# Ascend-Research/HeadPoseEstimation-WHENet

Measured on AMD Instinct MI355X. Metric: head crops/sec (224x224), higher is better.
Workload: dtype f16

## Files before the change

headposeestimation-whenet_amd/csrc/engine.cpp:

```cpp
#include "engine_internal.h"

#include <mutex>

#include <algorithm>
#include <cstdlib>
#include <cmath>
#include <cstring>

namespace whenet {

using namespace detail;

void* Engine::upload_bytes(const void* p, size_t nbytes) {
    weight_allocs_.emplace_back();
    weight_allocs_.back().reset(nbytes);
    void* d = weight_allocs_.back().as<void>();
    if (nbytes) WHENET_HIP_CHECK(hipMemcpy(d, p, nbytes, hipMemcpyHostToDevice));
    return d;
}

template <typename T> T* Engine::upload(const std::vector<T>& v) {
    return static_cast<T*>(upload_bytes(v.data(), v.size() * sizeof(T)));
}

// ... 170 lines not shown
        head_fuse_ = value != 0;
    } else if (key == "concurrent") {
        xcd_always_ = value != 0;
    } else if (key == "xcd_map") {
        WHENET_REQUIRE(value >= 0 && value <= 7, WHENET_EINVAL, "xcd_map must be a bit mask 0..7 (1 = front / front2, 2 = front7, 4 = head7)");
        xcd_map_ = int(value);
    } else if (key == "mb7") {
        mb7_ = value != 0;
    } else if (key == "front7") {
        front7_ = value != 0;
    } else if (key == "fold12") {
        fold12_ = value != 0;
    } else if (key == "front2_static") {
        WHENET_REQUIRE(value == 0 || value == 1, WHENET_EINVAL, "front2_static must be 0 (runtime tile geometry everywhere) or 1 (per layer, default)");
        front2_static_ = value != 0;
    } else if (key == "front_static") {
        WHENET_REQUIRE(value == 0 || value == 1, WHENET_EINVAL, "front_static must be 0 (runtime tile geometry everywhere) or 1 (per layer, default)");
        front_static_ = value != 0;
    } else if (key == "pw_static") {
        WHENET_REQUIRE(value == 0 || value == 1, WHENET_EINVAL, "pw_static must be 0 (runtime layer shapes everywhere) or 1 (per layer, default)");
        pw_static_ = value != 0;
    } else if (key == "stem_fuse") {
        stem_fuse_ = value != 0;
    } else if (key == "act_layout") {
        WHENET_REQUIRE(value >= 0 && value <= 2, WHENET_EINVAL,
                       "act_layout must be 0 (NHWC everywhere), 1 (16-channel blocks per layer, default) or 2 (16-channel blocks wherever supported)");
        act_layout_ = int(value);
    } else if (key == "poison") {
        poison_ = value != 0;
        return;
// ... 231 lines not shown
    } else {
        const DevBlock& c = blocks_[size_t(index)];
        const BlockSchedule cs = block_schedule(c);
        if (cs.use_mb7 || !cs.use_f7) return false;
        if (c.spec.has_skip() && c.project.K < 320) return false;
    }
    static constexpr bool WINS[17] = {false, false, false, false, false, false, false, false, false, false, false, false,
                                      true, true, true, true, true};
    return act_layout_ == 2 || (index <= 16 && WINS[index]);
}

bool Engine::front2_static(int index) const {
    static constexpr bool WINS[17] = {false, false, true, true, true, true, false, true, true, true, true, true, true,
                                      false, false, false, false};
    return front2_static_ && index >= 0 && index <= 16 && WINS[index];
}

bool Engine::pw_static(int index) const {
    static constexpr bool WINS[17] = {false, false, true, true, true, false, false, true, false, true, false, false, false,
                                      true, true, true, true};
    return pw_static_ && se_fuse_ == 1 && index >= 0 && index <= 16 && WINS[index];
}

bool Engine::front_static(int index) const {
    static constexpr bool WINS[17] = {false, false, false, false, false, false, true, false, false, false, false, false, false,
                                      false, false, false, false};
    return front_static_ && index >= 0 && index <= 16 && WINS[index];
}

void* Engine::enqueue_blocks(int first, int last, const View& v, void* cur, int n, hipStream_t s, LaunchRecorder* rec,
// ... 109 lines not shown
        fill_front_tiled(a, b);
        a.wep = b.expand.wp;
        a.wdt = b.dw.wt;
        if (fold == 2) {
            a.wep = d_fold12_w32_;
            a.be = fold12_pw_.bias;
            a.Cin = fold12_pw_.K;
            a.KSe = fold12_pw_.KS;
            a.NTe = fold12_pw_.NTILES;
            a.in_gate = static_cast<const float*>(v.gate);
        }
        a.xcd_grouped = xcd_grouped(1, n);
        a.plan = b.f2plan;
        a.plan.threads = front2_threads(b.f2plan, n);
        a.static_form = front2_static(sp.index);
        R(p + "/front", "front",
          kernel_name_front2(sp.k, sp.s, a.KSe, a.plan.threads, a.plan.xs, a.in_gate != nullptr, front2_static_row(a)).c_str(),
          bytes(a.Cin), flops(a.Cin), [&] { launch_front2(a, s); });
    } else if (bs.use_f2s) {
        Front2sArgs a{};
        fill_front_common(a, b, v, in, n);
        fill_front_tiled(a, b);
        a.weps = b.expand.wps;
        a.wdt = b.dw.wts;
        a.KSe = b.expand.KSs;
        a.wsi = b.expand.wsi;
        a.wsi_d = b.dw.wts_wsi;
        a.tm = b.f2s_tm;
        a.plan = b.f2splan;
        R(p + "/front", "front", kernel_name_front2s(sp.k, sp.s, a.KSe, a.plan.threads, a.tm, false).c_str(), bytes(a.Cin),
          flops(a.Cin), [&] { launch_front2s(a, s); });
    } else {
// ... 594 lines not shown
```

headposeestimation-whenet_amd/csrc/engine.h:

```cpp
#pragma once

#include <deque>
#include <map>
#include <memory>
#include <string>
#include <tuple>
#include <utility>
#include <vector>

#include "common.h"
#include "kernels.h"
#include "snapshot.h"

namespace whenet {

template <typename H, hipError_t (*Destroy)(H)>
class Owned {
  public:
    Owned() = default;
    Owned(Owned&& o) noexcept : h_(o.h_) { o.h_ = nullptr; }
    ~Owned() { reset(); }
    void reset() {
        if (h_) (void)Destroy(h_);
        h_ = nullptr;
// ... 357 lines not shown
    void enqueue_project(const DevBlock& b, const SeFuse& sef, bool se_fused, const View& v, const void* in, void* out, int n,
                         hipStream_t s, LaunchRecorder* rec, bool in_blocked, bool out_blocked);
    template <typename A> void fill_front_common(A& a, const DevBlock& b, const View& v, const void* in, int n) const;
    Head7Args head7_args(const void* x, float* feat, int n) const;
    PwArgs head_pw_args(const void* x, void* out, int n) const { return pw_args(head_, x, out, n * 49, 49, ACT_SWISH); }
    void* enqueue_blocks(int first, int last, const View& v, void* cur, int n, hipStream_t s, LaunchRecorder* rec,
                         bool b1_dw_done = false);
    bool stem_fuse_active() const;
    bool fold12_active() const;
    bool head_fused() const;
    bool heads_split_active() const;
    void launch_heads_stage(const HeadsArgs& h, const View& v, hipStream_t s);
    bool act_blocked(int index) const;
    bool front_static(int index) const;
    bool pw_static(int index) const;
    bool front2_static(int index) const;
    int act_layout_ = 1;
    struct BlockSchedule {
        bool fused = false, use_f2 = false, use_f2s = false, use_f7 = false, se_in_front = false, se_fused = false, se_mfma = false;
        bool use_mb7 = false;
        int se_ntiles = 1, se_chunks = 1;
    };
    BlockSchedule block_schedule(const DevBlock& b, int n = 0) const;
    int se_fuse_tiny_ = 0;
    int f2s_mask_ = -1;
    bool single_stage_call_ = false;
    bool range_call_ = false;
    int lanes_for(int n, int want) const;
    template <typename F> void for_each_lane(int n, int lanes, hipStream_t s, F&& body);
    void enqueue_lanes(const uint8_t* d_in, int n, Results out, hipStream_t s, int want = 0);
// ... 96 lines not shown
    bool fuse_front_ = true;
    int se_fuse_ = 1;
    int front_impl_ = 1;
    bool poison_ = false;
    bool head_fuse_ = true;
    bool front7_ = true;
    bool mb7_ = false;
    int xcd_map_ = 7;
    bool xcd_always_ = false;
    bool xcd_grouped(int bit, int n) const {
        return (xcd_map_ & bit) != 0 && (xcd_always_ || n >= 128);
    }
    bool stem_fuse_ = true;
    bool front_static_ = true;
    bool pw_static_ = true;
    bool front2_static_ = true;
    bool fold12_ = true;
    int lanes_ = 2;
    bool lane_graphs_ = false;
    int min_lane_crops_ = 16;
    int host_lanes_ = 2;
    Stream stream_, copy_stream_;
    std::vector<Stream> lane_streams_;
    std::vector<Event> join_ev_;
    Event fork_ev_;
    hipDeviceProp_t prop_{};
    int64_t params_backbone_ = 0, params_heads_ = 0;
    int n_tensors_ = 0;

    std::vector<DeviceBuffer> weight_allocs_;
// ... 60 lines not shown
```

headposeestimation-whenet_amd/csrc/front2.hip:

```cpp
#include "device_math.h"
#include "kernels.h"
#include "stamps.h"

#include <atomic>
#include <cstdlib>
#include <string>
#include <vector>

namespace whenet {

namespace {

constexpr int RL = 7;

__device__ __forceinline__ int fdiv2(int q, float rinv) { return int((float(q) + 0.5f) * rinv); }

struct F2Params {
    const half_t* x;
    const half_t* wep;
    const float* be;
    const half_t* wdt;
    const float* bd;
    half_t* out;
    float* rpart;
// ... 48 lines not shown
    g.chunks = cdiv(t.Cexp, g.CC);
    g.EH = (t.TH - 1) * t.s + t.k;
    g.EWp = 4 * (t.s * (t.TXG - 1) + nch);
    g.RP = g.EWp * 2;
    int cp = g.EH * g.RP + 8;
    cp = (cp + 63) / 64 * 64;
    g.CP = (cp - 32 >= g.EH * g.RP + 8) ? cp - 32 : cp + 32;
    const int ncq = cdiv((t.TH / RL) * t.TXG, 4);
    g.off_stage = (g.CC * g.CP + 15) & ~15;
    g.off_red = g.off_stage + (t.threads / 64) * 2048;
    g.off_sum = g.off_red + ncq * g.CC * 4;
    g.lds_bytes = g.off_sum + g.CC * 4;
    return g;
}

template <bool EDGE>
__device__ __forceinline__ void expand_store(const float16v& acc, float bias, unsigned char* ep, const int (&eoff)[4],
                                             const int (&drd)[4], const int (&dcd)[4], int nr_left, int ng_left) {
    (void)bias;
#pragma unroll
    for (int qq = 0; qq < 4; ++qq) {
        if (!EDGE || (drd[qq] < nr_left && dcd[qq] < ng_left)) {
            const float2v y0 = swish2(float2v{acc[4 * qq], acc[4 * qq + 1]});
            const float2v y1 = swish2(float2v{acc[4 * qq + 2], acc[4 * qq + 3]});
            half4 o;
            o[0] = half_t(y0[0]);
            o[1] = half_t(y0[1]);
            o[2] = half_t(y1[0]);
            o[3] = half_t(y1[1]);
            *reinterpret_cast<half4*>(ep + eoff[qq]) = o;
        }
    }
}

template <int K, int S, int KS, int NTHR, int XS, bool GATED, int ROW>
__device__ __forceinline__ void front2_body(const F2Params p) {
    constexpr F2Shape sg = f2_static_shape(ROW < 0 ? 0 : ROW);
    static_assert(ROW < 0 || (sg.k == K && sg.s == S && sg.KS == KS && sg.threads == NTHR && sg.xs == XS && (sg.gated != 0) == GATED),
                  "front2: the static plan belongs to another instantiation");
#define GEO(f) (ROW >= 0 ? sg.f : p.f)
    constexpr bool ONE_TILE = ROW >= 0 && sg.CC <= 32;
    constexpr int NCH = (3 * S + K + XS + 3) / 4;
    constexpr int NER = (RL - 1) * S + K;
    constexpr int NWAVE = NTHR / 64;
    constexpr int PF = KS <= 7 ? KS : 6;

    extern __shared__ __attribute__((aligned(16))) unsigned char smem[];
    unsigned char* E = smem;

    const int tid = threadIdx.x;
    const int lane = tid & 63;
    const int wave = __builtin_amdgcn_readfirstlane(tid >> 6);
    const int g = lane >> 5, lm = lane & 31;
    int b, tile, chunk;
    xcd_front(int(blockIdx.x), GEO(ntiles), GEO(chunks), p.n, p.xcd != 0, b, tile, chunk);
    const int tyi = tile / GEO(tiles_x), txi = tile - tyi * GEO(tiles_x);
    const int c0 = chunk * GEO(CC);
    const int ccur = (ROW >= 0 && sg.Cexp % sg.CC == 0) ? sg.CC
                                                        : ((GEO(Cexp) - c0 < GEO(CC)) ? (GEO(Cexp) - c0) : GEO(CC));
    const int H = GEO(H), Cin = GEO(Cin), RP = GEO(RP), CP = GEO(CP);
    const int oy0 = tyi * GEO(TH), ox0 = txi * GEO(TXG) * 4;
    const int iy0 = oy0 * S - GEO(pad), ix0 = ox0 * S - GEO(pad) - XS;

    const int er_lo = iy0 < 0 ? -iy0 : 0, er_hi = (iy0 + GEO(EH) < H) ? GEO(EH) : H - iy0;
    const int ex_lo = ix0 < 0 ? -ix0 : 0, ex_hi = (ix0 + GEO(EWp) < H) ? GEO(EWp) : H - ix0;
    const int g_lo = ex_lo >> 2, g_hi = (ex_hi + 3) >> 2;
    const int NG = g_hi - g_lo, NR = er_hi - er_lo;
    const int SCL = NG <= 2 ? 1 : (NG <= 4 ? 2 : 3), SC = 1 << SCL, SRL = 3 - SCL, SR = 1 << SRL;
    const int nsc = (NG + SC - 1) >> SCL, nsr = (NR + SR - 1) >> SRL;
    const int nstrip = nsc * nsr, ntile = (ccur + 31) >> 5, ntask = nstrip * ntile;

    const unsigned char* xb = reinterpret_cast<const unsigned char*>(p.x + size_t(b) * H * H * Cin);
    const half8* wf0 = reinterpret_cast<const half8*>(p.wep) + size_t(c0 >> 5) * 64 + lane;

    const int ua = lm >> 2;
    const int pixoff_a = (ua >> SCL) * H + 4 * (ua & (SC - 1)) + (lm & 3);
    int eoff[4], drd[4], dcd[4];
#pragma unroll
    for (int qq = 0; qq < 4; ++qq) {
        const int u = 2 * qq + g;
        drd[qq] = u >> SCL;
        dcd[qq] = u & (SC - 1);
        eoff[qq] = drd[qq] * RP + dcd[qq] * 8;
    }
    const int npix1 = H * H - 1;
// ... 45 lines not shown
    };
    const bool ktail = (Cin & 15) != 0 && g == 1;
    auto load_a = [&](half8 (&a)[PF], unsigned off, int ks0) {
#pragma unroll
        for (int u = 0; u < PF; ++u)
            if (ks0 + u < KS) a[u] = *reinterpret_cast<const half8*>(xb + off + (ks0 + u) * 32);
    };
    auto zero_ktail = [&](half8 (&a)[PF], int ks0) {
#pragma unroll
        for (int u = 0; u < PF; ++u)
            if (ks0 + u == KS - 1 && ktail) a[u] = half8{0, 0, 0, 0, 0, 0, 0, 0};
    };
    STAMP(0);
    int tl = 0, rb = 0, cbk = 0;
    int ti = t_begin, rbi = 0, cbki = 0;
    unsigned aoffq[D];
    auto issue = [&](int slot) {
        if (ti < t_end) {
            aoffq[slot] = a_offset(rbi, cbki);
            load_a(aq[slot], aoffq[slot], 0);
        }
        ++ti;
        if (++cbki == nsc) {
            cbki = 0;
            if (++rbi == nsr) rbi = 0;
        }
    };
    const bool fix_l = ex_lo > 0, fix_r = GEO(EWp) > ex_hi;
    if (t_begin < t_end) {
        tl = ONE_TILE ? 0 : __builtin_amdgcn_readfirstlane(t_begin / nstrip);
        const int st = t_begin - tl * nstrip;
        rb = __builtin_amdgcn_readfirstlane(st / nsc);
        cbk = st - rb * nsc;
        rbi = rb;
        cbki = cbk;
        load_w(tl);
#pragma unroll
        for (int d = 0; d < D; ++d) issue(d);
    }
    {
        const int nz = er_lo + (GEO(EH) - er_hi);
        if (nz > 0) {
            const float r_nz = __builtin_amdgcn_rcpf(float(nz));
            for (int pr = tid; pr < ccur * nz; pr += NTHR) {
                const int c = fdiv2(pr, r_nz), hr = pr - c * nz;
                const int er = hr < er_lo ? hr : er_hi + (hr - er_lo);
                unsigned char* rowp = E + c * CP + ((c >> 3) & 1) * 8 + er * RP;
                for (int q = 0; q < RP; q += 8) *reinterpret_cast<half4*>(rowp + q) = half4{0, 0, 0, 0};
            }
        }
    }

    STAMP(1);
    for (int t0 = t_begin; t0 < t_end; t0 += D) {
#pragma unroll
      for (int d = 0; d < D; ++d) {
        const int t = t0 + d;
        if (t >= t_end) break;
        float16v acc;
        zero_ktail(aq[d], 0);
        acc = __builtin_amdgcn_mfma_f32_32x32x16_f16(aq[d][0], w[0], bias16, 0, 0, 0);
#pragma unroll
        for (int u = 1; u < PF; ++u) acc = __builtin_amdgcn_mfma_f32_32x32x16_f16(aq[d][u], w[u], acc, 0, 0, 0);
#pragma unroll
        for (int ks = PF; ks < KS; ks += PF) {
            load_a(aq[d], aoffq[d], ks);
            zero_ktail(aq[d], ks);
#pragma unroll
            for (int u = 0; u < PF; ++u)
                if (ks + u < KS) acc = __builtin_amdgcn_mfma_f32_32x32x16_f16(aq[d][u], w[ks + u], acc, 0, 0, 0);
        }
        const int ch = tl * 32 + lm;
        unsigned char* ep = E + ch * CP + ((ch >> 3) & 1) * 8 + (er_lo + (rb << SRL)) * RP + (g_lo + (cbk << SCL)) * 8;
        unsigned char* ep0 = ep;
        const int nr_left = NR - (rb << SRL), ng_left = NG - (cbk << SCL), cbk_this = cbk;
        const float bias = bias_cur;
        int tln = tl;
        if (++cbk == nsc) {
            cbk = 0;
            if (++rb == nsr) {
                rb = 0;
                if (!ONE_TILE) ++tln;
            }
        }
        issue(d);
        if (!ONE_TILE && t + 1 < t_end && tln != tl) load_w(tln);
        tl = tln;
        if (ch < ccur) {
            if (nr_left >= SR && ng_left >= SC) expand_store<false>(acc, bias, ep, eoff, drd, dcd, nr_left, ng_left);
            else expand_store<true>(acc, bias, ep, eoff, drd, dcd, nr_left, ng_left);
        }
        if (ch < ccur) {
            if (fix_l && cbk_this == 0) {
#pragma unroll
                for (int dd = 0; dd < 2; ++dd) {
                    const int dr = g + 2 * dd;
                    if (dr < SR && dr < nr_left) {
// ... 10 lines not shown
                    const int dr = g + 2 * dd;
                    if (dr < SR && dr < nr_left) {
                        half_t* rowp = reinterpret_cast<half_t*>(ep0 + dr * RP) - 4 * (g_lo + cbk_this * SC) + ex_hi;
#pragma unroll
                        for (int q = 0; q < 8; ++q)
                            if (ex_hi + q < GEO(EWp)) rowp[q] = half_t(0);
                    }
                }
            }
        }
      }
    }

    STAMP(2);
    const int ncb = (ccur + 15) >> 4;
    const int ncol = (GEO(TH) / RL) * GEO(TXG), ncq = (ncol + 3) >> 2, nitem = ncb * ncq;
    const float r_txg = __builtin_amdgcn_rcpf(float(GEO(TXG)));
    const int i_begin = (wave * nitem) / NWAVE, i_end = ((wave + 1) * nitem) / NWAVE;
    const int cl = lane >> 2, j = lane & 3;
    half4 A[K][NCH];
    float bdv = 0.f;
    auto load_taps = [&](int cb) {
        const half4* src = reinterpret_cast<const half4*>(p.wdt) + (size_t((c0 >> 4) + cb) * K * NCH) * 64 + lane;
#pragma unroll
        for (int ky = 0; ky < K; ++ky)
#pragma unroll
            for (int ch = 0; ch < NCH; ++ch) A[ky][ch] = src[(ky * NCH + ch) * 64];
        bdv = p.bd[c0 + cb * 16 + cl];
    };
    int cb = 0, cq = 0;
    if (i_begin < i_end) {
        cb = __builtin_amdgcn_readfirstlane(i_begin / ncq);
        cq = i_begin - cb * ncq;
        load_taps(cb);
    }
    lds_barrier();
    STAMP(3);
    constexpr int W1V = 16;
    float w1v[W1V];
    {
        const int jo = tid >> 2, q = tid & 3;
#pragma unroll
        for (int i = 0; i < W1V; ++i) w1v[i] = 0.f;
        if (p.w1t != nullptr && wave * 16 < GEO(RPse)) {
            const float* wrow = p.w1t + size_t(jo < GEO(R) ? jo : GEO(R) - 1) * GEO(Cexp) + c0;
#pragma unroll
            for (int i = 0; i < W1V; ++i) {
                const int c = q + 4 * i;
                w1v[i] = wrow[c < ccur ? c : ccur - 1];
            }
        }
    }
    unsigned char* stg = smem + GEO(off_stage) + wave * 2048;
    float* s_red = reinterpret_cast<float*>(smem + GEO(off_red));
    float* s_sum = reinterpret_cast<float*>(smem + GEO(off_sum));
    const int jP = (lane >> 1) & 3, iP = (lane >> 3) & 3, hP = lane & 1, rP = lane >> 5;
    unsigned char* outb = reinterpret_cast<unsigned char*>(p.out + size_t(b) * GEO(Ho) * GEO(Ho) * GEO(Cexp));
    const unsigned row_bytes = unsigned(GEO(Ho)) * unsigned(GEO(Cexp)) * 2u;

    for (int it = i_begin; it < i_end; ++it) {
        const int col = cq * 4 + j;
        const int colc = col < ncol ? col : ncol - 1;
        const int seg = fdiv2(colc, r_txg), xgl = colc - seg * GEO(TXG);
        const int c = cb * 16 + cl;
        const unsigned char* bp = E + c * CP + ((c >> 3) & 1) * 8 + (seg * RL * S) * RP + xgl * (8 * S);
        float4v acc[RL];
        const float4v bd4 = float4v{bdv, bdv, bdv, bdv};
        bool started[RL];
#pragma unroll
        for (int r = 0; r < RL; ++r) started[r] = false;
#pragma unroll
        for (int er = 0; er < NER; ++er) {
            half4 bv[NCH];
#pragma unroll
            for (int ch = 0; ch < NCH; ++ch) bv[ch] = *reinterpret_cast<const half4*>(bp + er * RP + ch * 8);
#pragma unroll
            for (int ky = 0; ky < K; ++ky) {
                const int d = er - ky;
                if (d >= 0 && d % S == 0 && d / S < RL) {
#pragma unroll
                    for (int ch = 0; ch < NCH; ++ch) {
                        acc[d / S] = __builtin_amdgcn_mfma_f32_4x4x4f16(A[ky][ch], bv[ch], started[d / S] ? acc[d / S] : bd4, 0, 0, 0);
                        started[d / S] = true;
                    }
                }
            }
        }
        const int cb_this = cb, cq_this = cq;
        if (++cq == ncq) {
            cq = 0;
            ++cb;
            if (it + 1 < i_end) load_taps(cb);
        }
        const bool okc = col < ncol;
        const int oxb = ox0 + 4 * xgl;
        float m[4];
#pragma unroll
        for (int i = 0; i < 4; ++i) m[i] = (okc && oxb + i < GEO(Ho)) ? 1.f : 0.f;
        const int colP = cq_this * 4 + jP;
        const int colPc = colP < ncol ? colP : ncol - 1;
        const int segP = fdiv2(colPc, r_txg), xglP = colPc - segP * GEO(TXG);
        const int oxP = ox0 + 4 * xglP + iP;
        const bool okP = colP < ncol && oxP < GEO(Ho);
        const unsigned obase = (__umul24(unsigned(oy0 + segP * RL + rP), unsigned(GEO(Ho))) + unsigned(oxP)) * unsigned(GEO(Cexp)) * 2u +
                               unsigned(c0 + cb_this * 16 + hP * 8) * 2u;
        float2v sum2 = {0.f, 0.f};
        const float2v m01 = {m[0], m[1]}, m23 = {m[2], m[3]};
        unsigned char* sw = stg + j * 32 + cl * 2;
#pragma unroll
        for (int half = 0; half < 2; ++half) {
            const int r0 = half * 4, nr = half ? 3 : 4;
#pragma unroll
            for (int r = 0; r < nr; ++r) {
                const float2v y01 = swish2(float2v{acc[r0 + r][0], acc[r0 + r][1]});
                const float2v y23 = swish2(float2v{acc[r0 + r][2], acc[r0 + r][3]});
                sum2 = y01 * m01 + sum2;
                sum2 = y23 * m23 + sum2;
                *reinterpret_cast<half_t*>(sw + (r * 4 + 0) * 128) = half_t(y01[0]);
                *reinterpret_cast<half_t*>(sw + (r * 4 + 1) * 128) = half_t(y01[1]);
                *reinterpret_cast<half_t*>(sw + (r * 4 + 2) * 128) = half_t(y23[0]);
                *reinterpret_cast<half_t*>(sw + (r * 4 + 3) * 128) = half_t(y23[1]);
            }
            wave_lds_sync();
#pragma unroll
            for (int pp = 0; pp < 2; ++pp) {
                const int rl = 2 * pp + rP;
                const half8 v = *reinterpret_cast<const half8*>(stg + (pp * 64 + lane) * 16);
                if (okP && rl < nr) *reinterpret_cast<half8*>(outb + obase + unsigned(r0 + 2 * pp) * row_bytes) = v;
            }
            wave_lds_sync();
        }
        float sum = sum2[0] + sum2[1];
        sum += quad_xor1(sum);
        sum += quad_xor2(sum);
        if (j == 0) s_red[cq_this * GEO(CC) + c] = sum;
    }
    STAMP(4);
    lds_barrier();
    STAMP(5);

    if (tid < ccur) {
        float t = 0.0f;
        for (int q = 0; q < ncq; ++q) t += s_red[q * GEO(CC) + tid];
        if (p.w1t == nullptr) p.rpart[(size_t(b) * GEO(ntiles) + tile) * GEO(Cexp) + c0 + tid] = t;
        s_sum[tid] = t;
    }
    if (p.w1t == nullptr) {
        STAMP(6);
        return;
    }
    lds_barrier();
    {
        const int jo = tid >> 2, q = tid & 3;
        if (jo < GEO(RPse)) {
            float accr = 0.0f;
            if (jo < GEO(R)) {
                const float* wrow = p.w1t + size_t(jo) * GEO(Cexp) + c0;
#pragma unroll
                for (int i = 0; i < W1V; ++i) {
                    const int c = q + 4 * i;
                    if (c < ccur) accr = fmaf(s_sum[c], w1v[i], accr);
                }
                for (int c = q + 4 * W1V; c < ccur; c += 4) accr = fmaf(s_sum[c], wrow[c], accr);
            }
            const float pair = accr + quad_xor1(accr);
            const float tot = pair + quad_xor2(pair);
            if (q == 0)
                p.rpart[((size_t(b) * GEO(ntiles) + tile) * GEO(chunks) + chunk) * GEO(RPse) + jo] = (jo < GEO(R)) ? tot : 0.0f;
        }
    }
    STAMP(6);
}
#undef GEO

template <int K, int S, int KS, int NTHR, int XS, bool GATED>
__global__ __launch_bounds__(NTHR) void whenet_front2_kernel(const F2Params p) {
    front2_body<K, S, KS, NTHR, XS, GATED, -1>(p);
}

template <int K, int S, int KS, int NTHR, int XS, bool GATED, int ROW>
__global__ __launch_bounds__(NTHR) void whenet_front2_static_kernel(const F2Params p) {
    front2_body<K, S, KS, NTHR, XS, GATED, ROW>(p);
}

}

namespace {

constexpr bool f2_has_static(int row) { return TUNED2[row].use != 0; }

const char* f2_static_mismatch(const F2Shape& g, const Front2Args& a) {
    const Front2Plan& pl = a.plan;
    struct Field { const char* name; long long want, got; };
    const Field fields[] = {
        {"H", g.H, a.H}, {"Ho", g.Ho, a.Ho}, {"Cin", g.Cin, a.Cin}, {"Cexp", g.Cexp, a.Cexp}, {"pad", g.pad, a.pad}, {"NTe", g.NTe, a.NTe},
        {"CC", g.CC, pl.CC}, {"TH", g.TH, pl.TH}, {"TXG", g.TXG, pl.TXG}, {"tiles_x", g.tiles_x, pl.tiles_x}, {"tiles_y", g.tiles_y, pl.tiles_y},
        {"EH", g.EH, pl.EH}, {"EWp", g.EWp, pl.EWp}, {"RP", g.RP, pl.RP}, {"CP", g.CP, pl.CP},
// ... 22 lines not shown
        if (g.k == a.k && g.s == a.s && g.H == a.H && g.Ho == a.Ho && g.Cin == a.Cin && g.Cexp == a.Cexp && g.pad == a.pad && g.NTe == a.NTe &&
            g.KS == a.KSe && g.R == a.R && (g.gated != 0) == (a.in_gate != nullptr) && g.CC == a.plan.CC && g.TH == a.plan.TH &&
            g.TXG == a.plan.TXG && g.xs == a.plan.xs && g.threads == a.plan.threads)
            return r;
    }
    return -1;
}

void front2_static_check(int row, const Front2Args& a) {
    WHENET_REQUIRE(row >= 0 && row < NTUNED2 && f2_has_static(row), WHENET_EINVAL, "front2: no static form for this row of the plan table");
    f2_static_require(f2_static_shape(row), a);
}

int front2_static_selftest(int row, int field, int delta) {
    WHENET_REQUIRE(row >= 0 && row < NTUNED2 && f2_has_static(row), WHENET_EINVAL, "front2: no static form for this row of the plan table");
    WHENET_REQUIRE(field >= -1 && field < int(sizeof(F2Shape) / sizeof(int)), WHENET_EINVAL, "front2: no such field");
    F2Shape g = f2_static_shape(row);
    Front2Args a{};
    a.k = g.k;  a.s = g.s;  a.H = g.H;  a.Ho = g.Ho;  a.Cin = g.Cin;  a.Cexp = g.Cexp;  a.pad = g.pad;  a.NTe = g.NTe;  a.KSe = g.KS;  a.R = g.R;
    a.in_gate = g.gated ? reinterpret_cast<const float*>(&g) : nullptr;
    a.plan = make_front2_plan(g.k, g.s, g.Ho, g.Cexp, TUNED2[row].CC, TUNED2[row].TH, TUNED2[row].TXG, TUNED2[row].threads, TUNED2[row].xs);
    if (field >= 0) reinterpret_cast<int*>(&g)[field] += delta;
    f2_static_require(g, a);
    return 0;
}

namespace {

struct OncePerDevice {
    std::atomic<bool> done[64];
    OncePerDevice() { for (auto& d : done) d.store(false, std::memory_order_relaxed); }
};

template <int K, int S, int KS, int NTHR, int XS = 0, bool GATED = false, int ROW = -1>
void launch_f2(const Front2Args& a, hipStream_t stream) {
    const auto kernel = [] {
        if constexpr (ROW >= 0) return &whenet_front2_static_kernel<K, S, KS, NTHR, XS, GATED, ROW>;
        else return &whenet_front2_kernel<K, S, KS, NTHR, XS, GATED>;
    }();
    const Front2Plan& pl = a.plan;
    F2Params p{};
    p.x = static_cast<const half_t*>(a.x);
    p.wep = static_cast<const half_t*>(a.wep);
    p.be = a.be;
    p.wdt = static_cast<const half_t*>(a.wdt);
    p.bd = a.bd;
    p.out = static_cast<half_t*>(a.out);
    p.rpart = a.rpart;
    p.w1t = a.w1t;
    p.in_gate = a.in_gate;
    p.H = a.H;  p.Ho = a.Ho;  p.Cin = a.Cin;  p.Cexp = a.Cexp;  p.pad = a.pad;  p.NTe = a.NTe;
    p.CC = pl.CC;  p.TH = pl.TH;  p.TXG = pl.TXG;  p.tiles_x = pl.tiles_x;
    p.EH = pl.EH;  p.EWp = pl.EWp;  p.RP = pl.RP;  p.CP = pl.CP;
    p.off_stage = pl.off_stage;  p.off_red = pl.off_red;  p.off_sum = pl.off_sum;
    p.R = a.R;  p.RPse = (a.R + 3) & ~3;
    p.ntiles = pl.tiles_x * pl.tiles_y;  p.chunks = pl.chunks;  p.n = a.n;  p.xcd = a.xcd_grouped ? 1 : 0;
    WHENET_REQUIRE(pl.lds_bytes <= 160 * 1024, WHENET_EINVAL, "front2: the tile plan needs more than 160 KB of LDS");
    static OncePerDevice attr;
    int dev = 0;
    WHENET_HIP_CHECK(hipGetDevice(&dev));
    if (dev >= 0 && dev < 64 && !attr.done[dev].load(std::memory_order_acquire)) {
        if constexpr (ROW >= 0) front2_static_check(ROW, a);
        WHENET_HIP_CHECK(hipFuncSetAttribute(reinterpret_cast<const void*>(kernel), hipFuncAttributeMaxDynamicSharedMemorySize, 160 * 1024));
        attr.done[dev].store(true, std::memory_order_release);
    }
    hipLaunchKernelGGL(kernel, dim3(unsigned(pl.tiles_x * pl.tiles_y) * unsigned(pl.chunks) * unsigned(a.n)), dim3(NTHR),
                       pl.lds_bytes, stream, p);
    WHENET_HIP_CHECK(hipGetLastError());
}

void launch_f2_static(int row, const Front2Args& a, hipStream_t stream) {
    switch (row) {
        case 0: launch_f2<3, 2, 2, 512, 0, true, 0>(a, stream); break;
        case 1: launch_f2<3, 1, 2, 256, 0, false, 1>(a, stream); break;
        case 2: launch_f2<5, 2, 2, 256, 0, false, 2>(a, stream); break;
        case 3: launch_f2<5, 1, 3, 256, 0, false, 3>(a, stream); break;
        case 5: launch_f2<3, 1, 5, 256, 0, false, 5>(a, stream); break;
        case 6: launch_f2<5, 1, 5, 256, 0, false, 6>(a, stream); break;
        case 7: launch_f2<5, 1, 7, 256, 0, false, 7>(a, stream); break;
        case 8: launch_f2<5, 2, 7, 256, 0, false, 8>(a, stream); break;
        default: throw Error(WHENET_EINVAL, "front2: no static form for this row of the plan table");
    }
}

template <int NTHR>
void launch_f2_shape(const Front2Args& a, hipStream_t stream) {
// ... 113 lines not shown

void launch_front2(const Front2Args& a, hipStream_t stream) {
    WHENET_REQUIRE(a.KSe == ceil_div(a.Cin, 16), WHENET_EINVAL, "front2: k-steps do not match Cin");
    WHENET_REQUIRE(a.in_gate == nullptr || (a.k == 3 && a.s == 2 && a.KSe == 2 && a.Cin == 32), WHENET_EINVAL,
                   "front2: the gated-input form exists for the 3x3 / stride-2 / Cin = 32 shape only");
    Front2Args b = a;
    if (b.plan.threads != 256) {
        b.plan = make_front2_plan(a.k, a.s, a.Ho, a.Cexp, a.plan.CC, a.plan.TH, a.plan.TXG, a.plan.threads, a.plan.xs);
    }
    const int row = front2_static_row(b);
    if (row >= 0) launch_f2_static(row, b, stream);
    else if (b.plan.threads == 512) launch_f2_shape<512>(b, stream);
    else launch_f2_shape<256>(b, stream);
}

std::string kernel_name_front2(int k, int s, int kse, int threads, int xs, bool gated, int static_row) {
    return std::string(static_row >= 0 ? "whenet_front2_static_kernel<" : "whenet_front2_kernel<") + std::to_string(k) + ", " +
           std::to_string(s) + ", " + std::to_string(kse) + ", " + std::to_string(threads) + ", " + std::to_string(xs) + ", " +
           (gated ? "true" : "false") + (static_row >= 0 ? ", " + std::to_string(static_row) : std::string()) + ">";
}

}
```

headposeestimation-whenet_amd/csrc/kernels.h:

```cpp
#pragma once

#include <string>
#include <vector>

#include "common.h"
#include "overlay_host.h"
#include "jpeg_host.h"
#include "jpeg_dec_host.h"
#include "jpeg_dec_seg_host.h"
#include "jpeg_dec_clip_host.h"
#include "jpeg_prog_host.h"
#include "yuvx_host.h"

namespace whenet {

struct StemArgs {
    const uint8_t* in;
    void* out;
    const float* w;
    const float* bias;
    const float* lut;
    int n;
    const float* in_f32 = nullptr;
};
// ... 204 lines not shown
struct Front2Args {
    const void* x;
    const void* wep;
    const float* be;
    const void* wdt;
    const float* bd;
    void* out;
    float* rpart;
    const float* w1t;
    const float* in_gate;
    int R;
    int k, s, H, Ho, Cin, Cexp, pad, KSe, NTe, n;
    Front2Plan plan;
    bool xcd_grouped = false;
    bool static_form = false;
};
void launch_front2(const Front2Args& a, hipStream_t stream);
std::string kernel_name_front2(int k, int s, int kse, int threads, int xs, bool gated, int static_row = -1);
int front2_static_row(const Front2Args& a);
void front2_static_check(int row, const Front2Args& a);
int front2_static_selftest(int row, int field, int delta);

struct Front2sArgs {
    const void* x;
    const void* weps;
    const float* be;
    const void* wdt;
    const float* bd;
    void* out;
    float* rpart;
    const float* w1t;
    int R;
    int k, s, H, Ho, Cin, Cexp, pad, KSe, NTe, n;
// ... 486 lines not shown
```

Measured before the change: 184,700.

## Process two crops per workgroup in front2 static kernel for late blocks

```diff
diff --git a/headposeestimation-whenet_amd/csrc/engine.cpp b/headposeestimation-whenet_amd/csrc/engine.cpp
--- a/headposeestimation-whenet_amd/csrc/engine.cpp
+++ b/headposeestimation-whenet_amd/csrc/engine.cpp
@@ -208,6 +208,13 @@
     } else if (key == "front2_static") {
         WHENET_REQUIRE(value == 0 || value == 1, WHENET_EINVAL, "front2_static must be 0 (runtime tile geometry everywhere) or 1 (per layer, default)");
         front2_static_ = value != 0;
+    } else if (key == "front2_pair") {
+        WHENET_REQUIRE(value >= 0 && value <= 2, WHENET_EINVAL,
+                       "front2_pair must be 0 (one crop per workgroup), 1 (two where the per-layer table says so, default) or 2 (two wherever the form exists)");
+        front2_pair_ = int(value);
+    } else if (key == "front2_pair_mask") {
+        WHENET_REQUIRE(value >= -1 && value < (1 << 17), WHENET_EINVAL, "front2_pair_mask must be -1 or a bit mask of blocks 7..12");
+        front2_pair_mask_ = int(value);
     } else if (key == "front_static") {
         WHENET_REQUIRE(value == 0 || value == 1, WHENET_EINVAL, "front_static must be 0 (runtime tile geometry everywhere) or 1 (per layer, default)");
         front_static_ = value != 0;
@@ -469,6 +476,15 @@
     static constexpr bool WINS[17] = {false, false, true, true, true, true, false, true, true, true, true, true, true,
                                       false, false, false, false};
     return front2_static_ && index >= 0 && index <= 16 && WINS[index];
+}
+
+bool Engine::front2_pair(int index) const {
+    static constexpr bool WINS[17] = {false, false, false, false, false, false, false, false, false, false, false, false, true,
+                                      false, false, false, false};
+    if (front2_pair_ == 0 || !front2_static(index)) return false;
+    if (index < 7 || index > 12) return false;
+    if (front2_pair_ == 1 && front2_pair_mask_ >= 0) return ((front2_pair_mask_ >> index) & 1) != 0;
+    return front2_pair_ == 2 || WINS[index];
 }
 
 bool Engine::pw_static(int index) const {
@@ -608,8 +624,9 @@
         a.plan = b.f2plan;
         a.plan.threads = front2_threads(b.f2plan, n);
         a.static_form = front2_static(sp.index);
+        a.pair = front2_pair(sp.index) ? 1 : 0;
         R(p + "/front", "front",
-          kernel_name_front2(sp.k, sp.s, a.KSe, a.plan.threads, a.plan.xs, a.in_gate != nullptr, front2_static_row(a)).c_str(),
+          kernel_name_front2(sp.k, sp.s, a.KSe, a.plan.threads, a.plan.xs, a.in_gate != nullptr, front2_static_row(a), front2_pair_lanes(a)).c_str(),
           bytes(a.Cin), flops(a.Cin), [&] { launch_front2(a, s); });
     } else if (bs.use_f2s) {
         Front2sArgs a{};
diff --git a/headposeestimation-whenet_amd/csrc/engine.h b/headposeestimation-whenet_amd/csrc/engine.h
--- a/headposeestimation-whenet_amd/csrc/engine.h
+++ b/headposeestimation-whenet_amd/csrc/engine.h
@@ -395,6 +395,7 @@
     bool act_blocked(int index) const;
     bool front_static(int index) const;
     bool pw_static(int index) const;
+    bool front2_pair(int index) const;
     bool front2_static(int index) const;
     int act_layout_ = 1;
     struct BlockSchedule {
@@ -521,6 +522,8 @@
     bool stem_fuse_ = true;
     bool front_static_ = true;
     bool pw_static_ = true;
+    int front2_pair_mask_ = -1;
+    int front2_pair_ = 1;
     bool front2_static_ = true;
     bool fold12_ = true;
     int lanes_ = 2;
diff --git a/headposeestimation-whenet_amd/csrc/front2.hip b/headposeestimation-whenet_amd/csrc/front2.hip
--- a/headposeestimation-whenet_amd/csrc/front2.hip
+++ b/headposeestimation-whenet_amd/csrc/front2.hip
@@ -86,6 +86,34 @@
     return g;
 }
 
+constexpr int PAIR2_LANES[] = {0, 0, 0, 0, 0, 256, 256, 256, 256, 0, 0};
+static_assert(sizeof(PAIR2_LANES) / sizeof(int) == sizeof(TUNED2) / sizeof(TUNED2[0]), "front2: one pair entry per row of the plan table");
+
+struct F2PairShape {
+    int has, threads, comb, ncq;
+    int nstage;
+    int off_e1, off_stage, off_red, off_sum, lds_bytes;
+};
+constexpr int F2_PAIR_FIELDS = int(sizeof(F2PairShape) / sizeof(int));
+
+constexpr F2PairShape f2_pair_shape(int row, int threads) {
+    const F2Shape g = f2_static_shape(row);
+    F2PairShape q{};
+    q.has = (TUNED2[row].use != 0 && g.ntiles == 1 && g.CC == 32 && g.Cexp % 32 == 0 && g.gated == 0) ? 1 : 0;
+    q.threads = threads;
+    const int ncol = (g.TH / RL) * g.TXG;
+    q.comb = ncol == 2 ? 1 : 0;
+    q.ncq = cdiv(ncol, 4);
+    const int nitem = (g.CC / 16) * q.ncq * (q.comb ? 1 : 2);
+    q.nstage = nitem < threads / 64 ? nitem : threads / 64;
+    q.off_e1 = g.off_stage;
+    q.off_stage = 2 * q.off_e1;
+    q.off_red = q.off_stage + q.nstage * 2048;
+    q.off_sum = q.off_red + 2 * q.ncq * g.CC * 4;
+    q.lds_bytes = q.off_sum + 2 * g.CC * 4;
+    return q;
+}
+
 template <bool EDGE>
 __device__ __forceinline__ void expand_store(const float16v& acc, float bias, unsigned char* ep, const int (&eoff)[4],
                                              const int (&drd)[4], const int (&dcd)[4], int nr_left, int ng_left) {
@@ -105,11 +133,15 @@
     }
 }
 
-template <int K, int S, int KS, int NTHR, int XS, bool GATED, int ROW>
+template <int K, int S, int KS, int NTHR, int XS, bool GATED, int ROW, bool PAIR = false>
 __device__ __forceinline__ void front2_body(const F2Params p) {
     constexpr F2Shape sg = f2_static_shape(ROW < 0 ? 0 : ROW);
-    static_assert(ROW < 0 || (sg.k == K && sg.s == S && sg.KS == KS && sg.threads == NTHR && sg.xs == XS && (sg.gated != 0) == GATED),
+    constexpr F2PairShape pg = f2_pair_shape(ROW < 0 ? 0 : ROW, NTHR);
+    static_assert(ROW < 0 || (sg.k == K && sg.s == S && sg.KS == KS && (PAIR || sg.threads == NTHR) && sg.xs == XS && (sg.gated != 0) == GATED),
                   "front2: the static plan belongs to another instantiation");
+    static_assert(!PAIR || (ROW >= 0 && pg.has != 0), "front2: this row of the plan table has no pair form");
+    constexpr bool COMB = PAIR && pg.comb != 0;
+    constexpr int NCR = (PAIR && !COMB) ? 2 : 1;
 #define GEO(f) (ROW >= 0 ? sg.f : p.f)
     constexpr bool ONE_TILE = ROW >= 0 && sg.CC <= 32;
     constexpr int NCH = (3 * S + K + XS + 3) / 4;
@@ -125,7 +157,14 @@
     const int wave = __builtin_amdgcn_readfirstlane(tid >> 6);
     const int g = lane >> 5, lm = lane & 31;
     int b, tile, chunk;
-    xcd_front(int(blockIdx.x), GEO(ntiles), GEO(chunks), p.n, p.xcd != 0, b, tile, chunk);
+    xcd_front(int(blockIdx.x), GEO(ntiles), GEO(chunks), PAIR ? (p.n + 1) >> 1 : p.n, p.xcd != 0, b, tile, chunk);
+    bool two = false;
+    unsigned xoffB = 0u;
+    if constexpr (PAIR) {
+        b *= 2;
+        two = b + 1 < p.n;
+        xoffB = two ? unsigned(sg.H * sg.H * sg.Cin) * 2u : 0u;
+    }
     const int tyi = tile / GEO(tiles_x), txi = tile - tyi * GEO(tiles_x);
     const int c0 = chunk * GEO(CC);
     const int ccur = (ROW >= 0 && sg.Cexp % sg.CC == 0) ? sg.CC
@@ -140,7 +179,7 @@
     const int NG = g_hi - g_lo, NR = er_hi - er_lo;
     const int SCL = NG <= 2 ? 1 : (NG <= 4 ? 2 : 3), SC = 1 << SCL, SRL = 3 - SCL, SR = 1 << SRL;
     const int nsc = (NG + SC - 1) >> SCL, nsr = (NR + SR - 1) >> SRL;
-    const int nstrip = nsc * nsr, ntile = (ccur + 31) >> 5, ntask = nstrip * ntile;
+    const int nstrip = nsc * nsr, ntile = (ccur + 31) >> 5, ntask = nstrip * ntile * (PAIR ? 2 : 1);
 
     const unsigned char* xb = reinterpret_cast<const unsigned char*>(p.x + size_t(b) * H * H * Cin);
     const half8* wf0 = reinterpret_cast<const half8*>(p.wep) + size_t(c0 >> 5) * 64 + lane;
@@ -216,22 +255,28 @@
     STAMP(0);
     int tl = 0, rb = 0, cbk = 0;
     int ti = t_begin, rbi = 0, cbki = 0;
+    int cr = 0, cri = 0;
     unsigned aoffq[D];
     auto issue = [&](int slot) {
         if (ti < t_end) {
             aoffq[slot] = a_offset(rbi, cbki);
+            if constexpr (PAIR) aoffq[slot] += cri ? xoffB : 0u;
             load_a(aq[slot], aoffq[slot], 0);
         }
         ++ti;
         if (++cbki == nsc) {
             cbki = 0;
-            if (++rbi == nsr) rbi = 0;
+            if (++rbi == nsr) {
+                rbi = 0;
+                if constexpr (PAIR) ++cri;
+            }
         }
     };
     const bool fix_l = ex_lo > 0, fix_r = GEO(EWp) > ex_hi;
     if (t_begin < t_end) {
         tl = ONE_TILE ? 0 : __builtin_amdgcn_readfirstlane(t_begin / nstrip);
-        const int st = t_begin - tl * nstrip;
+        if constexpr (PAIR) cr = cri = (t_begin >= nstrip) ? 1 : 0;
+        const int st = t_begin - (PAIR ? cr : tl) * nstrip;
         rb = __builtin_amdgcn_readfirstlane(st / nsc);
         cbk = st - rb * nsc;
         rbi = rb;
@@ -244,10 +289,18 @@
         const int nz = er_lo + (GEO(EH) - er_hi);
         if (nz > 0) {
             const float r_nz = __builtin_amdgcn_rcpf(float(nz));
-            for (int pr = tid; pr < ccur * nz; pr += NTHR) {
-                const int c = fdiv2(pr, r_nz), hr = pr - c * nz;
+            for (int pr = tid; pr < ccur * nz * (PAIR ? 2 : 1); pr += NTHR) {
+                int c = fdiv2(pr, r_nz);
+                const int hr = pr - c * nz;
                 const int er = hr < er_lo ? hr : er_hi + (hr - er_lo);
-                unsigned char* rowp = E + c * CP + ((c >> 3) & 1) * 8 + er * RP;
+                unsigned char* rowp = E;
+                if constexpr (PAIR) {
+                    if (c >= ccur) {
+                        c -= ccur;
+                        rowp += pg.off_e1;
+                    }
+                }
+                rowp += c * CP + ((c >> 3) & 1) * 8 + er * RP;
                 for (int q = 0; q < RP; q += 8) *reinterpret_cast<half4*>(rowp + q) = half4{0, 0, 0, 0};
             }
         }
@@ -273,7 +326,7 @@
                 if (ks + u < KS) acc = __builtin_amdgcn_mfma_f32_32x32x16_f16(aq[d][u], w[ks + u], acc, 0, 0, 0);
         }
         const int ch = tl * 32 + lm;
-        unsigned char* ep = E + ch * CP + ((ch >> 3) & 1) * 8 + (er_lo + (rb << SRL)) * RP + (g_lo + (cbk << SCL)) * 8;
+        unsigned char* ep = E + (PAIR && cr ? pg.off_e1 : 0) + ch * CP + ((ch >> 3) & 1) * 8 + (er_lo + (rb << SRL)) * RP + (g_lo + (cbk << SCL)) * 8;
         unsigned char* ep0 = ep;
         const int nr_left = NR - (rb << SRL), ng_left = NG - (cbk << SCL), cbk_this = cbk;
         const float bias = bias_cur;
@@ -283,6 +336,7 @@
             if (++rb == nsr) {
                 rb = 0;
                 if (!ONE_TILE) ++tln;
+                if constexpr (PAIR) ++cr;
             }
         }
         issue(d);
@@ -323,7 +377,7 @@
 
     STAMP(2);
     const int ncb = (ccur + 15) >> 4;
-    const int ncol = (GEO(TH) / RL) * GEO(TXG), ncq = (ncol + 3) >> 2, nitem = ncb * ncq;
+    const int ncol = (GEO(TH) / RL) * GEO(TXG), ncq = (ncol + 3) >> 2, nitem = ncb * ncq * NCR;
     const float r_txg = __builtin_amdgcn_rcpf(float(GEO(TXG)));
     const int i_begin = (wave * nitem) / NWAVE, i_end = ((wave + 1) * nitem) / NWAVE;
     const int cl = lane >> 2, j = lane & 3;
@@ -337,10 +391,14 @@
             for (int ch = 0; ch < NCH; ++ch) A[ky][ch] = src[(ky * NCH + ch) * 64];
         bdv = p.bd[c0 + cb * 16 + cl];
     };
-    int cb = 0, cq = 0;
+    int cb = 0, cq = 0, icr = 0;
     if (i_begin < i_end) {
-        cb = __builtin_amdgcn_readfirstlane(i_begin / ncq);
-        cq = i_begin - cb * ncq;
+        cb = __builtin_amdgcn_readfirstlane(i_begin / (ncq * NCR));
+        cq = i_begin - cb * (ncq * NCR);
+        if constexpr (NCR == 2) {
+            icr = cq >= ncq ? 1 : 0;
+            cq -= icr * ncq;
+        }
         load_taps(cb);
     }
     lds_barrier();
@@ -348,10 +406,16 @@
     constexpr int W1V = 16;
     float w1v[W1V];
     {
-        const int jo = tid >> 2, q = tid & 3;
+        int jo = tid >> 2;
+        const int q = tid & 3;
 #pragma unroll
         for (int i = 0; i < W1V; ++i) w1v[i] = 0.f;
-        if (p.w1t != nullptr && wave * 16 < GEO(RPse)) {
+        const int waveh = PAIR ? (wave >= NWAVE / 2 ? wave - NWAVE / 2 : wave) : wave;
+        if constexpr (PAIR) {
+            const int th = tid & (NTHR / 2 - 1);
+            jo = th >> 2;
+        }
+        if (p.w1t != nullptr && waveh * 16 < GEO(RPse)) {
             const float* wrow = p.w1t + size_t(jo < GEO(R) ? jo : GEO(R) - 1) * GEO(Cexp) + c0;
 #pragma unroll
             for (int i = 0; i < W1V; ++i) {
@@ -360,19 +424,23 @@
             }
         }
     }
-    unsigned char* stg = smem + GEO(off_stage) + wave * 2048;
-    float* s_red = reinterpret_cast<float*>(smem + GEO(off_red));
-    float* s_sum = reinterpret_cast<float*>(smem + GEO(off_sum));
+    unsigned char* stg = smem + (PAIR ? pg.off_stage : GEO(off_stage)) + ((PAIR && pg.nstage < NWAVE) ? i_begin : wave) * 2048;
+    float* s_red = reinterpret_cast<float*>(smem + (PAIR ? pg.off_red : GEO(off_red)));
+    float* s_sum = reinterpret_cast<float*>(smem + (PAIR ? pg.off_sum : GEO(off_sum)));
     const int jP = (lane >> 1) & 3, iP = (lane >> 3) & 3, hP = lane & 1, rP = lane >> 5;
     unsigned char* outb = reinterpret_cast<unsigned char*>(p.out + size_t(b) * GEO(Ho) * GEO(Ho) * GEO(Cexp));
     const unsigned row_bytes = unsigned(GEO(Ho)) * unsigned(GEO(Cexp)) * 2u;
+    const unsigned ooffB = unsigned(GEO(Ho) * GEO(Ho)) * unsigned(GEO(Cexp)) * 2u;
+    float zf = 0.f;
+    if constexpr (COMB) asm volatile("" : "+v"(zf));
 
     for (int it = i_begin; it < i_end; ++it) {
-        const int col = cq * 4 + j;
+        const int col = COMB ? (j & 1) : cq * 4 + j;
         const int colc = col < ncol ? col : ncol - 1;
         const int seg = fdiv2(colc, r_txg), xgl = colc - seg * GEO(TXG);
         const int c = cb * 16 + cl;
-        const unsigned char* bp = E + c * CP + ((c >> 3) & 1) * 8 + (seg * RL * S) * RP + xgl * (8 * S);
+        const int crj = COMB ? (j >> 1) : icr;
+        const unsigned char* bp = E + (PAIR && crj ? pg.off_e1 : 0) + c * CP + ((c >> 3) & 1) * 8 + (seg * RL * S) * RP + xgl * (8 * S);
         float4v acc[RL];
         const float4v bd4 = float4v{bdv, bdv, bdv, bdv};
         bool started[RL];
@@ -395,25 +463,31 @@
                 }
             }
         }
-        const int cb_this = cb, cq_this = cq;
+        const int cb_this = cb, cq_this = cq, icr_this = icr;
         if (++cq == ncq) {
             cq = 0;
-            ++cb;
-            if (it + 1 < i_end) load_taps(cb);
+            if (NCR == 1 || ++icr == NCR) {
+                icr = 0;
+                ++cb;
+                if (it + 1 < i_end) load_taps(cb);
+            }
         }
         const bool okc = col < ncol;
         const int oxb = ox0 + 4 * xgl;
         float m[4];
 #pragma unroll
         for (int i = 0; i < 4; ++i) m[i] = (okc && oxb + i < GEO(Ho)) ? 1.f : 0.f;
-        const int colP = cq_this * 4 + jP;
+        const int colP = COMB ? (jP & 1) : cq_this * 4 + jP;
         const int colPc = colP < ncol ? colP : ncol - 1;
         const int segP = fdiv2(colPc, r_txg), xglP = colPc - segP * GEO(TXG);
         const int oxP = ox0 + 4 * xglP + iP;
-        const bool okP = colP < ncol && oxP < GEO(Ho);
+        const int crP = COMB ? (jP >> 1) : icr_this;
+        const bool okP = colP < ncol && oxP < GEO(Ho) && (!PAIR || crP == 0 || two);
         const unsigned obase = (__umul24(unsigned(oy0 + segP * RL + rP), unsigned(GEO(Ho))) + unsigned(oxP)) * unsigned(GEO(Cexp)) * 2u +
-                               unsigned(c0 + cb_this * 16 + hP * 8) * 2u;
+                               unsigned(c0 + cb_this * 16 + hP * 8) * 2u + (PAIR && crP ? ooffB : 0u);
         float2v sum2 = {0.f, 0.f};
+        float2v dup2 = {0.f, 0.f};
+        const float2v z2 = {zf, zf};
         const float2v m01 = {m[0], m[1]}, m23 = {m[2], m[3]};
         unsigned char* sw = stg + j * 32 + cl * 2;
 #pragma unroll
@@ -425,6 +499,10 @@
                 const float2v y23 = swish2(float2v{acc[r0 + r][2], acc[r0 + r][3]});
                 sum2 = y01 * m01 + sum2;
                 sum2 = y23 * m23 + sum2;
+                if constexpr (COMB) {
+                    dup2 = y01 * z2 + dup2;
+                    dup2 = y23 * z2 + dup2;
+                }
                 *reinterpret_cast<half_t*>(sw + (r * 4 + 0) * 128) = half_t(y01[0]);
                 *reinterpret_cast<half_t*>(sw + (r * 4 + 1) * 128) = half_t(y01[1]);
                 *reinterpret_cast<half_t*>(sw + (r * 4 + 2) * 128) = half_t(y23[0]);
@@ -440,15 +518,31 @@
             wave_lds_sync();
         }
         float sum = sum2[0] + sum2[1];
-        sum += quad_xor1(sum);
-        sum += quad_xor2(sum);
-        if (j == 0) s_red[cq_this * GEO(CC) + c] = sum;
+        if constexpr (COMB) {
+            float dd = dup2[0] + dup2[1];
+            dd += dd;
+            sum += quad_xor1(sum);
+            sum += quad_xor1(dd);
+            if ((j & 1) == 0) s_red[crj * pg.ncq * GEO(CC) + c] = sum;
+        } else {
+            sum += quad_xor1(sum);
+            sum += quad_xor2(sum);
+            if (j == 0) s_red[(PAIR ? icr_this * pg.ncq : 0) * GEO(CC) + cq_this * GEO(CC) + c] = sum;
+        }
     }
     STAMP(4);
     lds_barrier();
     STAMP(5);
 
-    if (tid < ccur) {
+    if constexpr (PAIR) {
+        if (tid < 2 * ccur) {
+            const int e = tid >= ccur ? 1 : 0, ch = tid - e * ccur;
+            float t = 0.0f;
+            for (int q = 0; q < ncq; ++q) t += s_red[(e * ncq + q) * GEO(CC) + ch];
+            if (p.w1t == nullptr && (e == 0 || two)) p.rpart[(size_t(b + e) * GEO(ntiles) + tile) * GEO(Cexp) + c0 + ch] = t;
+            s_sum[e * GEO(CC) + ch] = t;
+        }
+    } else if (tid < ccur) {
         float t = 0.0f;
         for (int q = 0; q < ncq; ++q) t += s_red[q * GEO(CC) + tid];
         if (p.w1t == nullptr) p.rpart[(size_t(b) * GEO(ntiles) + tile) * GEO(Cexp) + c0 + tid] = t;
@@ -460,7 +554,9 @@
     }
     lds_barrier();
     {
-        const int jo = tid >> 2, q = tid & 3;
+        const int e = (PAIR && tid >= NTHR / 2) ? 1 : 0, th = PAIR ? (tid & (NTHR / 2 - 1)) : tid;
+        const int jo = th >> 2, q = th & 3;
+        const float* ssum = s_sum + e * GEO(CC);
         if (jo < GEO(RPse)) {
             float accr = 0.0f;
             if (jo < GEO(R)) {
@@ -468,14 +564,14 @@
 #pragma unroll
                 for (int i = 0; i < W1V; ++i) {
                     const int c = q + 4 * i;
-                    if (c < ccur) accr = fmaf(s_sum[c], w1v[i], accr);
+                    if (c < ccur) accr = fmaf(ssum[c], w1v[i], accr);
                 }
-                for (int c = q + 4 * W1V; c < ccur; c += 4) accr = fmaf(s_sum[c], wrow[c], accr);
+                for (int c = q + 4 * W1V; c < ccur; c += 4) accr = fmaf(ssum[c], wrow[c], accr);
             }
             const float pair = accr + quad_xor1(accr);
             const float tot = pair + quad_xor2(pair);
-            if (q == 0)
-                p.rpart[((size_t(b) * GEO(ntiles) + tile) * GEO(chunks) + chunk) * GEO(RPse) + jo] = (jo < GEO(R)) ? tot : 0.0f;
+            if (q == 0 && (e == 0 || two))
+                p.rpart[((size_t(b + e) * GEO(ntiles) + tile) * GEO(chunks) + chunk) * GEO(RPse) + jo] = (jo < GEO(R)) ? tot : 0.0f;
         }
     }
     STAMP(6);
@@ -490,6 +586,12 @@
 template <int K, int S, int KS, int NTHR, int XS, bool GATED, int ROW>
 __global__ __launch_bounds__(NTHR) void whenet_front2_static_kernel(const F2Params p) {
     front2_body<K, S, KS, NTHR, XS, GATED, ROW>(p);
+}
+
+template <int K, int S, int KS, int NTHR, int XS, bool GATED, int ROW, int PAIR>
+__global__ __launch_bounds__(NTHR * PAIR) void whenet_front2_static_kernel(const F2Params p) {
+    static_assert(PAIR == 1 || PAIR == 2, "front2: pair workgroups have NTHR or 2 NTHR lanes");
+    front2_body<K, S, KS, NTHR * PAIR, XS, GATED, ROW, true>(p);
 }
 
 }
@@ -542,7 +644,10 @@
 
 int front2_static_selftest(int row, int field, int delta) {
     WHENET_REQUIRE(row >= 0 && row < NTUNED2 && f2_has_static(row), WHENET_EINVAL, "front2: no static form for this row of the plan table");
-    WHENET_REQUIRE(field >= -1 && field < int(sizeof(F2Shape) / sizeof(int)), WHENET_EINVAL, "front2: no such field");
+    constexpr int NF = int(sizeof(F2Shape) / sizeof(int));
+    if (field >= NF) return front2_pair_selftest(row, field - NF, delta);
+    if (field == -1 && PAIR2_LANES[row] != 0) front2_pair_selftest(row, -1, 0);
+    WHENET_REQUIRE(field >= -1, WHENET_EINVAL, "front2: no such field");
     F2Shape g = f2_static_shape(row);
     Front2Args a{};
     a.k = g.k;  a.s = g.s;  a.H = g.H;  a.Ho = g.Ho;  a.Cin = g.Cin;  a.Cexp = g.Cexp;  a.pad = g.pad;  a.NTe = g.NTe;  a.KSe = g.KS;  a.R = g.R;
@@ -553,6 +658,72 @@
     return 0;
 }
 
+Front2PairPlan make_front2_pair_plan(const Front2Plan& p, int Cexp, int threads) {
+    Front2PairPlan q;
+    const int ncol = (p.TH / RL) * p.TXG;
+    q.has = (p.tiles_x == 1 && p.tiles_y == 1 && p.CC == 32 && Cexp % 32 == 0 && (threads == 256 || threads == 512)) ? 1 : 0;
+    q.threads = threads;
+    q.comb = ncol == 2 ? 1 : 0;
+    q.ncq = ceil_div(ncol, 4);
+    const int nitem = ceil_div(p.CC, 16) * q.ncq * (q.comb ? 1 : 2);
+    q.nstage = nitem < threads / 64 ? nitem : threads / 64;
+    q.off_e1 = int((size_t(p.CC) * p.CP + 15) & ~size_t(15));
+    q.off_stage = 2 * q.off_e1;
+    q.off_red = q.off_stage + q.nstage * 2048;
+    q.off_sum = q.off_red + 2 * q.ncq * p.CC * 4;
+    q.lds_bytes = size_t(q.off_sum) + 2 * size_t(p.CC) * 4;
+    return q;
+}
+
+namespace {
+
+constexpr bool f2_has_pair(int row) { return PAIR2_LANES[row] != 0 && f2_pair_shape(row, PAIR2_LANES[row]).has != 0; }
+
+void f2_pair_require(const F2PairShape& g, const Front2Args& a) {
+    const Front2PairPlan q = make_front2_pair_plan(a.plan, a.Cexp, g.threads);
+    struct Field { const char* name; long long want, got; };
+    const Field fields[] = {
+        {"has", g.has, q.has}, {"threads", g.threads, q.threads}, {"comb", g.comb, q.comb}, {"ncq", g.ncq, q.ncq}, {"nstage", g.nstage, q.nstage}, {"off_e1", g.off_e1, q.off_e1},
+        {"off_stage", g.off_stage, q.off_stage}, {"off_red", g.off_red, q.off_red}, {"off_sum", g.off_sum, q.off_sum},
+        {"lds_bytes", g.lds_bytes, (long long)q.lds_bytes},
+    };
+    static_assert(sizeof(fields) / sizeof(fields[0]) == F2_PAIR_FIELDS, "front2: every field of the pair plan is compared");
+    for (const Field& f : fields)
+        if (f.want != f.got) throw Error(WHENET_EINVAL, std::string("front2: the static pair plan differs from the runtime plan in field ") + f.name);
+    WHENET_REQUIRE(g.has == 1 && (g.threads == 256 || g.threads == 512) && g.lds_bytes <= 160 * 1024, WHENET_EINVAL,
+                   "front2: no pair form for this plan");
+}
+
+}
+
+void front2_pair_check(int row, int threads, const Front2Args& a) {
+    WHENET_REQUIRE(row >= 0 && row < NTUNED2 && f2_has_static(row) && PAIR2_LANES[row] != 0, WHENET_EINVAL,
+                   "front2: no pair form for this row of the plan table");
+    front2_static_check(row, a);
+    f2_pair_require(f2_pair_shape(row, threads), a);
+}
+
+int front2_pair_selftest(int row, int field, int delta) {
+    WHENET_REQUIRE(row >= 0 && row < NTUNED2 && f2_has_static(row) && f2_has_pair(row), WHENET_EINVAL,
+                   "front2: no pair form for this row of the plan table");
+    WHENET_REQUIRE(field >= -1 && field < F2_PAIR_FIELDS, WHENET_EINVAL, "front2: no such field");
+    const F2Shape g = f2_static_shape(row);
+    F2PairShape q = f2_pair_shape(row, PAIR2_LANES[row]);
+    Front2Args a{};
+    a.Cexp = g.Cexp;
+    a.plan = make_front2_plan(g.k, g.s, g.Ho, g.Cexp, TUNED2[row].CC, TUNED2[row].TH, TUNED2[row].TXG, TUNED2[row].threads, TUNED2[row].xs);
+    if (field >= 0) reinterpret_cast<int*>(&q)[field] += delta;
+    f2_pair_require(q, a);
+    return 0;
+}
+
+int front2_pair_lanes(const Front2Args& a) {
+    if (a.pair == 0) return 0;
+    const int row = front2_static_row(a);
+    if (row < 0 || !f2_has_pair(row)) return 0;
+    return a.pair == 1 ? PAIR2_LANES[row] : a.pair;
+}
+
 namespace {
 
 struct OncePerDevice {
@@ -560,10 +731,12 @@
     OncePerDevice() { for (auto& d : done) d.store(false, std::memory_order_relaxed); }
 };
 
-template <int K, int S, int KS, int NTHR, int XS = 0, bool GATED = false, int ROW = -1>
+template <int K, int S, int KS, int NTHR, int XS = 0, bool GATED = false, int ROW = -1, int PAIR = 0>
 void launch_f2(const Front2Args& a, hipStream_t stream) {
+    static_assert(PAIR == 0 || ROW >= 0, "front2: the pair form is a static form");
     const auto kernel = [] {
-        if constexpr (ROW >= 0) return &whenet_front2_static_kernel<K, S, KS, NTHR, XS, GATED, ROW>;
+        if constexpr (PAIR != 0) return &whenet_front2_static_kernel<K, S, KS, NTHR, XS, GATED, ROW, PAIR>;
+        else if constexpr (ROW >= 0) return &whenet_front2_static_kernel<K, S, KS, NTHR, XS, GATED, ROW>;
         else return &whenet_front2_kernel<K, S, KS, NTHR, XS, GATED>;
     }();
     const Front2Plan& pl = a.plan;
@@ -588,16 +761,39 @@
     int dev = 0;
     WHENET_HIP_CHECK(hipGetDevice(&dev));
     if (dev >= 0 && dev < 64 && !attr.done[dev].load(std::memory_order_acquire)) {
-        if constexpr (ROW >= 0) front2_static_check(ROW, a);
+        if constexpr (PAIR != 0) front2_pair_check(ROW, NTHR * PAIR, a);
+        else if constexpr (ROW >= 0) front2_static_check(ROW, a);
         WHENET_HIP_CHECK(hipFuncSetAttribute(reinterpret_cast<const void*>(kernel), hipFuncAttributeMaxDynamicSharedMemorySize, 160 * 1024));
         attr.done[dev].store(true, std::memory_order_release);
     }
-    hipLaunchKernelGGL(kernel, dim3(unsigned(pl.tiles_x * pl.tiles_y) * unsigned(pl.chunks) * unsigned(a.n)), dim3(NTHR),
-                       pl.lds_bytes, stream, p);
+    if constexpr (PAIR != 0) {
+        const Front2PairPlan q = make_front2_pair_plan(pl, a.Cexp, NTHR * PAIR);
+        WHENET_REQUIRE(q.has == 1 && q.lds_bytes <= 160 * 1024, WHENET_EINVAL, "front2: no pair form for this plan");
+        hipLaunchKernelGGL(kernel, dim3(unsigned(pl.chunks) * unsigned((a.n + 1) / 2)), dim3(NTHR * PAIR), q.lds_bytes, stream, p);
+    } else {
+        hipLaunchKernelGGL(kernel, dim3(unsigned(pl.tiles_x * pl.tiles_y) * unsigned(pl.chunks) * unsigned(a.n)), dim3(NTHR),
+                           pl.lds_bytes, stream, p);
+    }
     WHENET_HIP_CHECK(hipGetLastError());
 }
 
 void launch_f2_static(int row, const Front2Args& a, hipStream_t stream) {
+    const int pl = front2_pair_lanes(a);
+    if (pl != 0) {
+        WHENET_REQUIRE(pl == 256 || pl == 512, WHENET_EINVAL, "front2: pair workgroups have 256 or 512 lanes");
+        switch (row * 2 + (pl == 512 ? 1 : 0)) {
+            case 10: launch_f2<3, 1, 5, 256, 0, false, 5, 1>(a, stream); break;
+            case 11: launch_f2<3, 1, 5, 256, 0, false, 5, 2>(a, stream); break;
+            case 12: launch_f2<5, 1, 5, 256, 0, false, 6, 1>(a, stream); break;
+            case 13: launch_f2<5, 1, 5, 256, 0, false, 6, 2>(a, stream); break;
+            case 14: launch_f2<5, 1, 7, 256, 0, false, 7, 1>(a, stream); break;
+            case 15: launch_f2<5, 1, 7, 256, 0, false, 7, 2>(a, stream); break;
+            case 16: launch_f2<5, 2, 7, 256, 0, false, 8, 1>(a, stream); break;
+            case 17: launch_f2<5, 2, 7, 256, 0, false, 8, 2>(a, stream); break;
+            default: throw Error(WHENET_EINVAL, "front2: no pair form for this row of the plan table");
+        }
+        return;
+    }
     switch (row) {
         case 0: launch_f2<3, 2, 2, 512, 0, true, 0>(a, stream); break;
         case 1: launch_f2<3, 1, 2, 256, 0, false, 1>(a, stream); break;
@@ -741,10 +937,11 @@
     else launch_f2_shape<256>(b, stream);
 }
 
-std::string kernel_name_front2(int k, int s, int kse, int threads, int xs, bool gated, int static_row) {
+std::string kernel_name_front2(int k, int s, int kse, int threads, int xs, bool gated, int static_row, int pair_lanes) {
     return std::string(static_row >= 0 ? "whenet_front2_static_kernel<" : "whenet_front2_kernel<") + std::to_string(k) + ", " +
            std::to_string(s) + ", " + std::to_string(kse) + ", " + std::to_string(threads) + ", " + std::to_string(xs) + ", " +
-           (gated ? "true" : "false") + (static_row >= 0 ? ", " + std::to_string(static_row) : std::string()) + ">";
-}
-
-}
+           (gated ? "true" : "false") + (static_row >= 0 ? ", " + std::to_string(static_row) : std::string()) +
+           (static_row >= 0 && pair_lanes > 0 ? ", " + std::to_string(pair_lanes / threads) : std::string()) + ">";
+}
+
+}
diff --git a/headposeestimation-whenet_amd/csrc/kernels.h b/headposeestimation-whenet_amd/csrc/kernels.h
--- a/headposeestimation-whenet_amd/csrc/kernels.h
+++ b/headposeestimation-whenet_amd/csrc/kernels.h
@@ -242,9 +242,22 @@
     Front2Plan plan;
     bool xcd_grouped = false;
     bool static_form = false;
-};
+    int pair = 0;
+};
+struct Front2PairPlan {
+    int has = 0, threads = 0;
+    int comb = 0;
+    int ncq = 0;
+    int nstage = 0;
+    int off_e1 = 0, off_stage = 0, off_red = 0, off_sum = 0;
+    size_t lds_bytes = 0;
+};
+Front2PairPlan make_front2_pair_plan(const Front2Plan& p, int Cexp, int threads);
 void launch_front2(const Front2Args& a, hipStream_t stream);
-std::string kernel_name_front2(int k, int s, int kse, int threads, int xs, bool gated, int static_row = -1);
+std::string kernel_name_front2(int k, int s, int kse, int threads, int xs, bool gated, int static_row = -1, int pair_lanes = 0);
+int front2_pair_lanes(const Front2Args& a);
+void front2_pair_check(int row, int threads, const Front2Args& a);
+int front2_pair_selftest(int row, int field, int delta);
 int front2_static_row(const Front2Args& a);
 void front2_static_check(int row, const Front2Args& a);
 int front2_static_selftest(int row, int field, int delta);
```

New measurement: 185,200, median of 6. Within noise of the previous version (+0.3%).
